# crockwell/far

Measured on AMD Instinct MI355X. Metric: image-pairs/sec (match+solve+regress) at 640x480, higher is better.
Workload: dtype f32

## Files before the change

### far_amd/csrc/conv_igemm_f16s.hip

```cpp
#include "common.h"
#include "linear_small.h"
#include <vector>
#include <type_traits>

namespace {

typedef _Float16 f16x8 __attribute__((ext_vector_type(8)));
typedef __attribute__((address_space(1))) const void* gptr_t;
typedef __attribute__((address_space(3))) void* lptr_t;

constexpr int TW = 16;
constexpr int A_PXB = 80;
constexpr int ACT_EXP_DEFAULT = 4;

template <int KS, int MW, int ST>
struct Geo {
    static constexpr int TH = 4 * MW;
    static constexpr int HW = ST * (TW - 1) + KS, HH = ST * (TH - 1) + KS;
    static constexpr int PX = KS == 1 ? 64 * MW : HW * HH;
    static constexpr int ROWB = KS == 1 ? 0 : (HW * A_PXB + 255) / 256 * 256;
    static constexpr int A_PLANE = KS == 1 ? PX * A_PXB : HH * ROWB;
    static constexpr int ITEMS = PX * 4;
    __device__ static constexpr int px_off(int hy, int hx) { return hy * ROWB + hx * A_PXB; }
};

struct ConvArgs {
    const float* x;
    const float* x2;
    int Cin1;
    const unsigned char* w;
    const float* zeros;
    const float* scale;
    const float* shift;
    const float* res;
    int res_group;
    const float* ln_gamma;
    const float* ln_beta;
    float ln_eps;
    const float* post_res;
    const float* up;
    float* y;
    long npix;
    long ntiles;
    int Csub;
    int H, W, Ho, Wo, Cin, Cout, tilesX, tilesY, nchunks, nblkY, act;
    float slope;
    float act_scale;
    float out_mul;
    int* overflow;
    const float* scale_dev;
    float* kv_part;
    int kv_S, kv_valid;
    const unsigned char* kv_img;
    float la_eps, la_vlen;
    int sub2;
    const long* g_b;
    const long* g_cell;
    int g_wc, g_W, g_stride, g_Hf, g_Wf;
};

__device__ __forceinline__ void split8(const float4& u, const float4& v, float act_scale, f16x8& hi, f16x8& lo) {
    const float x[8] = {u.x, u.y, u.z, u.w, v.x, v.y, v.z, v.w};
#pragma unroll
    for (int i = 0; i < 8; i += 2) {
        f16x2 h, l;
        split2(f32x2{x[i], x[i + 1]} * f32x2{act_scale, act_scale}, h, l);
        hi[i] = h.x; hi[i + 1] = h.y;
        lo[i] = l.x; lo[i + 1] = l.y;
    }
}

typedef float f32x4 __attribute__((ext_vector_type(4)));
template <int ITERS>
struct Stage {
    f32x4 v[ITERS][2];
};

struct TilePos {
    int img, oy0, ox0;
    long pix0;
};

template <int KS, int MW, int ST, int NTHR, int ITERS>
__device__ __forceinline__ void stage_pixels(int (&pixv)[ITERS], const ConvArgs& p, const TilePos& tp, int tid) {
    using G = Geo<KS, MW, ST>;
#pragma unroll
    for (int it = 0; it < ITERS; ++it) {
        const int i = tid + NTHR * it;
        const int hp = i >> 2;
        const int hy = hp / G::HW, hx = hp - hy * G::HW;
        const int iy = ST * tp.oy0 - KS / 2 + hy, ix = ST * tp.ox0 - KS / 2 + hx;
        const bool ok = i < G::ITEMS && iy >= 0 && iy < p.H && ix >= 0 && ix < p.W;
        pixv[it] = ok ? (tp.img * p.H + iy) * p.W + ix : -1;
    }
}

template <int KS, int MW, int ST, int NTHR, int ITERS>
__device__ __forceinline__ void stage_load(Stage<ITERS>& st, const ConvArgs& p, const TilePos& tp, int chunk, int tid, bool live = true,
                                           const int* rowpix = nullptr, const int* pixv = nullptr) {
    using G = Geo<KS, MW, ST>;
#pragma unroll
    for (int it = 0; it < ITERS; ++it) {
        const int i = tid + NTHR * it;
        const int hp = i >> 2, g = i & 3;
        const int c0 = 32 * chunk + 8 * g;
        bool ok = live && i < G::ITEMS;
        long pix;
        if (KS != 1 && pixv) {
            pix = pixv[it];
            ok = live && pixv[it] >= 0;
        } else if (KS == 1) {
            pix = tp.pix0 + hp;
            ok = ok && pix < p.npix;
            if (rowpix) {
                const int gp = rowpix[hp < 64 * MW ? hp : 0];
                pix = gp;
                ok = ok && gp >= 0;
            } else if (p.sub2) {
                const unsigned up = (unsigned)pix, rowg = up / (unsigned)p.Wo, ox = up - rowg * (unsigned)p.Wo;
                const unsigned n = rowg / (unsigned)p.Ho, oy = rowg - n * (unsigned)p.Ho;
                pix = ((long)n * p.H + 2 * oy) * p.W + 2 * ox;
            }
        } else {
            const int hy = hp / G::HW, hx = hp - hy * G::HW;
            const int iy = ST * tp.oy0 - KS / 2 + hy, ix = ST * tp.ox0 - KS / 2 + hx;
            ok = ok && iy >= 0 && iy < p.H && ix >= 0 && ix < p.W;
            pix = ((long)tp.img * p.H + iy) * p.W + ix;
        }
        const bool ok0 = ok && c0 < p.Cin, ok1 = ok && c0 + 4 < p.Cin;
#if defined(FAR_K9_EXP) && (FAR_K9_EXP & 4)
        pix &= 1023;
#endif
        const bool second = c0 >= p.Cin1;
        const float* base = second ? p.x2 + pix * (p.Cin - p.Cin1) + (c0 - p.Cin1) : p.x + pix * p.Cin1 + c0;
#if defined(FAR_K9_EXP) && (FAR_K9_EXP & 1)
        const float* src0 = p.zeros;
        const float* src1 = p.zeros;
        (void)base; (void)ok0; (void)ok1;
#else
        const float* src0 = ok0 ? base : p.zeros;
        const float* src1 = ok1 ? base + 4 : p.zeros;
#endif
        asm volatile("global_load_dwordx4 %0, %1, off" : "=v"(st.v[it][0]) : "v"(src0) : "memory");
        asm volatile("global_load_dwordx4 %0, %1, off" : "=v"(st.v[it][1]) : "v"(src1) : "memory");
    }
}

template <int YOUNGER, int ITERS>
__device__ __forceinline__ void stage_arrived(Stage<ITERS>& st) {
    static_assert(YOUNGER >= 0 && YOUNGER < 64, "vmcnt is a 6-bit counter");
    asm volatile("s_waitcnt vmcnt(%0)" : : "n"(YOUNGER) : "memory");
#pragma unroll
    for (int it = 0; it < ITERS; ++it) {
        f32x4 &u = st.v[it][0], &w = st.v[it][1];
        asm volatile("" : "+v"(u), "+v"(w));
    }
}

template <int KS, int MW, int ST, int NTHR, int ITERS, bool SPLIT>
__device__ __forceinline__ void stage_store(const Stage<ITERS>& st, unsigned char* As, int tid, float act_scale) {
    using G = Geo<KS, MW, ST>;
#pragma unroll
    for (int it = 0; it < ITERS; ++it) {
        const int i = tid + NTHR * it;
        const float4 u = make_float4(st.v[it][0].x, st.v[it][0].y, st.v[it][0].z, st.v[it][0].w);
        const float4 w = make_float4(st.v[it][1].x, st.v[it][1].y, st.v[it][1].z, st.v[it][1].w);
        if (ITERS * NTHR == G::ITEMS || i < G::ITEMS) {
            const int hp = i >> 2, g = i & 3;
            int off;
            if (KS == 1) off = hp * A_PXB;
            else { const int hy = hp / G::HW; off = G::px_off(hy, hp - hy * G::HW); }
            f16x8 hi, lo;
            split8(u, w, act_scale, hi, lo);
            *reinterpret_cast<f16x8*>(As + off + g * 16) = hi;
            if (SPLIT) *reinterpret_cast<f16x8*>(As + G::A_PLANE + off + g * 16) = lo;
        }
    }
}

template <int KS, int NTW>
__device__ __forceinline__ void conv_epilogue(const ConvArgs& p, const f32x16 (&acc)[2][NTW], const TilePos& tp,
                                              int cout_w, int wm, int l31, int h) {
    const float* __restrict__ resp = p.res;
    float* __restrict__ yp = p.y;
    const int rowstep = (KS == 1 ? 16 : p.Wo) * p.Csub;
#pragma unroll
    for (int mt = 0; mt < 2; ++mt) {
        const int mtile = 2 * wm + mt;
        long pix0;
        int nrow, ncol;
        if (KS == 1) {
            pix0 = tp.pix0 + 32 * mtile;
            const long left = p.npix - pix0;
            nrow = left >= 32 ? 2 : (left > 16 ? 2 : (left > 0 ? 1 : 0));
            ncol = left >= 32 ? 16 : -1;
        } else {
            const int oy = tp.oy0 + 2 * mtile;
            pix0 = ((long)tp.img * p.Ho + oy) * p.Wo + tp.ox0;
            nrow = p.Ho - oy;
            ncol = p.Wo - tp.ox0;
        }
        const long left = KS == 1 ? p.npix - pix0 : 0;
        int delta[16];
        bool ok[16];
#pragma unroll
        for (int r = 0; r < 16; ++r) {
            const int trow = r >> 3, tcol = (r & 3) + 8 * ((r >> 2) & 1) + 4 * h;
            delta[r] = trow * rowstep + tcol * p.Csub;
            ok[r] = (KS == 1 && ncol < 0) ? (16 * trow + tcol < left) : (trow < nrow && tcol < ncol);
        }
#pragma unroll
        for (int nt = 0; nt < NTW; ++nt) {
            const int co = cout_w + 32 * nt + l31;
            if (co >= p.Cout) continue;
            const float sc = p.scale[co] * p.out_mul, sh = p.shift ? p.shift[co] : 0.f;
            const int plane = co / p.Csub;
            const long base = (long)plane * p.npix * p.Csub + pix0 * p.Csub + (co - plane * p.Csub);
            float rv[16];
#pragma unroll
            for (int r = 0; r < 16; ++r) {
                rv[r] = 0.f;
                if (resp && ok[r]) {
                    if (p.res_group > 1) {
                        const long pix = pix0 + 16 * (r >> 3) + ((r & 3) + 8 * ((r >> 2) & 1) + 4 * h);
                        rv[r] = resp[(pix / p.res_group) * p.Cout + co];
                    } else {
                        rv[r] = resp[base + delta[r]];
                    }
                }
            }
#pragma unroll
            for (int r = 0; r < 16; ++r) {
                float v = acc[mt][nt][r] * sc + sh + rv[r];
                if (p.act == 1) v = fmaxf(v, 0.f);
                else if (p.act == 2) v = v > 0.f ? v : v * p.slope;
                if (ok[r]) yp[base + delta[r]] = v;
            }
        }
    }
}

#if defined(FAR_K9_EXP) && (FAR_K9_EXP & 8)
#define FAR_K9_STORE4(ptr, val) __builtin_nontemporal_store(f32x4{(val).x, (val).y, (val).z, (val).w}, reinterpret_cast<f32x4*>(ptr))
#else
#define FAR_K9_STORE4(ptr, val) (*reinterpret_cast<float4*>(ptr) = (val))
#endif

#ifdef FAR_K9_TIMING
__device__ unsigned long long g_k9_stamps[12 * 65536];
#define FAR_K9_STAMP(i) do { if (threadIdx.x == 0 && blockIdx.x < 65536) g_k9_stamps[12 * blockIdx.x + (i)] = __builtin_amdgcn_s_memtime(); } while (0)
#else
#define FAR_K9_STAMP(i) do {} while (0)
#endif

#define FAR_DPP_F(v, ctrl) __builtin_bit_cast(float, __builtin_amdgcn_update_dpp(0, __builtin_bit_cast(int, v), ctrl, 0xF, 0xF, true))
__device__ __forceinline__ float sum32(float v) {
    v += FAR_DPP_F(v, 0xB1);
    v += FAR_DPP_F(v, 0x4E);
    v += FAR_DPP_F(v, 0x141);
    v += FAR_DPP_F(v, 0x140);
    return v + shfl_xor_f(v, 16);
}

__device__ __forceinline__ void arrived(float4& v) { asm volatile("" : "+v"(v.x), "+v"(v.y), "+v"(v.z), "+v"(v.w)); }

template <int KS, int NW, int UP>
__device__ __forceinline__ void conv_epilogue_wide(const ConvArgs& p, const f32x16 (&acc)[2][4], const TilePos& tp,
                                                   int cout_w, int wm, int wave, int lane, float* lw, float* xch,
                                                   int mask_mt = -1, int mask_lo = 0, int mask_hi = 0) {
    const int l31 = lane & 31, h = lane >> 5;
    const float* __restrict__ resp = p.res;
    float* __restrict__ yp = p.y;
    float sc[4], sh[4];
#pragma unroll
    for (int nt = 0; nt < 4; ++nt) {
        const int co = cout_w + 32 * nt + l31;
        sc[nt] = co < p.Cout ? p.scale[co] * p.out_mul : 0.f;
        sh[nt] = (co < p.Cout && p.shift) ? p.shift[co] : 0.f;
    }
    const int co4 = cout_w + 4 * l31;
    const bool cok_all = co4 < p.Cout;
    const bool lane_masked = l31 >= mask_lo && l31 < mask_hi;
    const int plane = cok_all ? co4 / p.Csub : 0;
    const long cbase = (long)plane * p.npix * p.Csub + (co4 - plane * p.Csub);
#pragma unroll
    for (int mt = 0; mt < 2; ++mt) {
        const bool cok = cok_all && !(mt == mask_mt && lane_masked);
        const int mtile = 2 * wm + mt;
        long pix0;
        int nrow, ncol;
        long left = 0;
        if (KS == 1) {
            pix0 = tp.pix0 + 32 * mtile;
            left = p.npix - pix0;
            nrow = 2; ncol = 16;
        } else {
            const int oy = tp.oy0 + 2 * mtile;
            pix0 = ((long)tp.img * p.Ho + oy) * p.Wo + tp.ox0;
            nrow = p.Ho - oy;
            ncol = p.Wo - tp.ox0;
        }
#pragma unroll
        for (int nt = 0; nt < 4; ++nt)
#pragma unroll
// ... 875 lines not shown
            float v = 0.f;
            if (n < Cout && ch < Cin) v = w[(long)n * s_co + (long)ch * s_ci + (long)tap * s_tap] * wmul;
            const _Float16 hh = (_Float16)v;
            dst[e] = hh;
            if (planes == 2) dst[(size_t)NT * 16 + e] = (_Float16)(v - (float)hh);
        }
    }
}

struct PackRow {
    const float* w;
    long s_co, s_ci, s_tap;
    int Cin, Cout, taps, nchunks, nblkY, NT, planes, owns_scale;
    const float* w_all;
    long n_all;
    float* pack_scale;
    _Float16* out;
    const float* base_scale;
    float* scale_vec;
};
__device__ AmaxSlot g_pack_slots[4096];

__global__ __launch_bounds__(256) void k_pack_table_scales(const PackRow* __restrict__ rows) {
    const PackRow r = rows[blockIdx.y];
    if (!r.owns_scale) return;
    __shared__ unsigned part[256];
    unsigned m = 0;
    for (long i = (long)blockIdx.x * 256 + threadIdx.x; i < r.n_all; i += (long)gridDim.x * 256) {
        const unsigned b = __float_as_uint(fabsf(r.w_all[i]));
        m = b > m ? b : m;
    }
    part[threadIdx.x] = m;
    __syncthreads();
    for (int d = 128; d >= 1; d >>= 1) {
        if ((int)threadIdx.x < d && part[threadIdx.x + d] > part[threadIdx.x]) part[threadIdx.x] = part[threadIdx.x + d];
        __syncthreads();
    }
    if (threadIdx.x == 0) {
        AmaxSlot* const sl = g_pack_slots + (blockIdx.y & 4095);
        atomicMax(&sl->max_bits, part[0]);
        __threadfence();
        if (atomicAdd(&sl->ticket, 1u) == gridDim.x - 1) {
            __threadfence();
            const unsigned bits = atomicExch(&sl->max_bits, 0u);
            atomicExch(&sl->ticket, 0u);
            write_scales<0>(__uint_as_float(bits), r.pack_scale);
        }
    }
}

__global__ __launch_bounds__(256) void k_pack_table_images(const PackRow* __restrict__ rows) {
    const PackRow r = rows[blockIdx.y];
    const float wmul = r.pack_scale[0];
    if (r.scale_vec && blockIdx.x == 0)
        for (int co = threadIdx.x; co < r.Cout; co += 256) r.scale_vec[co] = (r.base_scale ? r.base_scale[co] : 1.0f) * r.pack_scale[1];
    const long total = (long)r.taps * r.nchunks * 2 * r.nblkY * r.NT * 2;
    if (blockIdx.x == 0 && threadIdx.x < 16) r.out[(size_t)total * 8 * r.planes + threadIdx.x] = (_Float16)0.f;
    for (long i = (long)blockIdx.x * 256 + threadIdx.x; i < total; i += (long)gridDim.x * 256) {
        long t = i;
        const int s = (int)(t & 1); t >>= 1;
        const int nn = (int)(t % r.NT); t /= r.NT;
        const int by = (int)(t % r.nblkY); t /= r.nblkY;
        const int ks = (int)(t & 1); t >>= 1;
        const int tap = (int)(t % r.taps);
        const int chunk = (int)(t / r.taps);
        const int n = by * r.NT + nn;
        const size_t row = r.planes == 2 ? ((((size_t)(chunk * r.taps + tap) * 2 + ks) * r.nblkY + by) * 2) * r.NT + nn
                                         : ((((size_t)(chunk * r.taps + tap) * r.nblkY + by) * 2 + ks)) * r.NT + nn;
        _Float16* dst = r.out + row * 16 + ((s ^ ((nn >> 3) & 1)) * 8);
        for (int e = 0; e < 8; ++e) {
            const int ch = 32 * chunk + 16 * ks + 8 * s + e;
            float v = 0.f;
            if (n < r.Cout && ch < r.Cin) v = r.w[(long)n * r.s_co + (long)ch * r.s_ci + (long)tap * r.s_tap] * wmul;
            const _Float16 hh = (_Float16)v;
            dst[e] = hh;
            if (r.planes == 2) dst[(size_t)r.NT * 16 + e] = (_Float16)(v - (float)hh);
        }
    }
}

struct TileCfg { int mw, nw, nt; };
inline TileCfg cfg_for(int Cout, int stride) {
    const int pad128 = (Cout + 127) / 128 * 128, pad256 = (Cout + 255) / 256 * 256;
    return (stride == 1 && pad128 < pad256) ? TileCfg{4, 1, 128} : TileCfg{2, 2, 256};
}

template <int KS, int MW, int NW, int NTW, bool SPLIT, int ST = 1, int UP = 0, bool N7 = false, int EPI = 0>
int launch_conv(const ConvArgs& a, dim3 grid, hipStream_t stream) {
    using G = Geo<KS, MW, ST>;
    constexpr int PLANES = SPLIT ? 2 : 1;
    constexpr int smem_loop = PLANES * G::A_PLANE + 3 * 2 * 32 * NTW * NW * 32;
    constexpr int smem_epi = EPI == 2 ? MW * NW * 32 * LDW * 4
                                      : MW * NW * (32 * 128 * 4 + 32 * 4);
    constexpr int smem_need = smem_loop + (EPI != 0 ? 64 * MW * 4 : 0);
    constexpr int smem = smem_need > smem_epi ? smem_need : smem_epi;
    bool cfg_failed = false;
    FAR_ONCE_PER_DEVICE(cfg_failed = hipFuncSetAttribute((const void*)k_conv<KS, MW, NW, NTW, SPLIT, ST, UP, N7, EPI>,
                                                         hipFuncAttributeMaxDynamicSharedMemorySize, smem) != hipSuccess);
    if (cfg_failed) return far_check_launch();
    hipLaunchKernelGGL((k_conv<KS, MW, NW, NTW, SPLIT, ST, UP, N7, EPI>), grid, dim3(64 * MW * NW), smem, stream, a);
    return far_check_launch();
}

template <int KS, bool SPLIT>
int launch_cfg(const TileCfg& c, const ConvArgs& a, dim3 grid, hipStream_t stream, bool small = false) {
    if (KS == 1 && a.up) {
        const bool rowwise = (a.Wo & 31) == 0 && far_get_tuning(13) == 0;
        if (c.mw == 4) return rowwise ? launch_conv<1, 4, 1, 4, SPLIT, 1, 2>(a, grid, stream) : launch_conv<1, 4, 1, 4, SPLIT, 1, 1>(a, grid, stream);
        return rowwise ? launch_conv<1, 2, 2, 4, SPLIT, 1, 2>(a, grid, stream) : launch_conv<1, 2, 2, 4, SPLIT, 1, 1>(a, grid, stream);
    }
    if constexpr (KS == 1) {
        if (c.mw == 2 && small) return launch_conv<1, 1, 2, 4, SPLIT>(a, grid, stream);
        if (c.mw == 4 && small) return launch_conv<1, 2, 1, 4, SPLIT>(a, grid, stream);
    }
    if (c.mw == 4) return launch_conv<KS, 4, 1, 4, SPLIT>(a, grid, stream);
    if constexpr (KS == 3) {
        if (a.nblkY == 1 && a.Cout > 192 && a.Cout <= 224 && ((a.Cout | a.Csub) & 3) == 0 && far_get_tuning(4) == 0)
            return launch_conv<KS, 2, 2, 4, SPLIT, 1, false, true>(a, grid, stream);
    }
    return launch_conv<KS, 2, 2, 4, SPLIT>(a, grid, stream);
}

template <bool SPLIT>
int launch_stride2(const ConvArgs& a, dim3 grid, hipStream_t stream) { return launch_conv<3, 2, 2, 4, SPLIT, 2>(a, grid, stream); }

}

extern "C" {

int far_weight_scale_f32(const float* w, long n, float* scale_out, hipStream_t stream);
int far_conv_pack_view_f32(const float* w, long s_co, long s_ci, long s_tap, int Cin, int Cout, int ksize, int stride, int split,
                           const float* scale_in, void* packed, hipStream_t stream);
int far_conv_pack_view_scaled_f32(const float* w, long s_co, long s_ci, long s_tap, int Cin, int Cout, int ksize, int stride, int split,
                                  const float* scale_in, void* packed, const float* base_scale, float* scale_vec_out,
                                  hipStream_t stream);

size_t far_conv_packed_bytes(int Cin, int Cout, int ksize, int stride, int split) {
    if (Cin <= 0 || Cout <= 0 || (ksize != 1 && ksize != 3) || stride < 1 || stride > 2 || (stride == 2 && ksize != 3)) return 0;
    const int NT = cfg_for(Cout, stride).nt;
    const size_t nchunks = (Cin + 31) / 32, nblkY = (Cout + NT - 1) / NT;
    return (size_t)ksize * ksize * nchunks * nblkY * (split ? 2 : 1) * NT * 64 + 32;
}

int far_conv_pack_f32(const float* w, int Cin, int Cout, int ksize, int stride, int w_exp, int split, void* packed,
                      hipStream_t stream) {
    far_clear_errors();
    if (!w || !packed || far_conv_packed_bytes(Cin, Cout, ksize, stride, split) == 0 || w_exp < -60 || w_exp > 60) return FAR_EINVAL;
    const int NT = cfg_for(Cout, stride).nt;
    const int nchunks = (Cin + 31) / 32, nblkY = (Cout + NT - 1) / NT;
    hipLaunchKernelGGL(k_conv_pack, dim3(512), dim3(256), 0, stream, w, (long)Cin * ksize * ksize, (long)ksize * ksize, 1L, Cin, Cout,
                       ksize * ksize, nchunks, nblkY, NT, split ? 2 : 1, ldexpf(1.0f, w_exp), (const float*)nullptr, (_Float16*)packed);
    return far_check_launch();
}

int far_weight_scale_f32(const float* w, long n, float* scale_out, hipStream_t stream) {
    far_clear_errors();
    if (!w || !scale_out || n <= 0) return FAR_EINVAL;
    if ((reinterpret_cast<uintptr_t>(w) & 15) == 0) {
        launch_amax_scale<0>(w, n, scale_out, stream);
    } else {
        hipMemsetAsync(scale_out, 0, 2 * sizeof(float), stream);
        hipLaunchKernelGGL(k_absmax_bits, dim3(256), dim3(256), 0, stream, w, n, reinterpret_cast<unsigned*>(scale_out));
        hipLaunchKernelGGL(k_pack_scale, dim3(1), dim3(1), 0, stream, scale_out);
    }
    return far_check_launch();
}

int far_conv_pack_view_f32(const float* w, long s_co, long s_ci, long s_tap, int Cin, int Cout, int ksize, int stride, int split,
                           const float* scale_in, void* packed, hipStream_t stream) {
    return far_conv_pack_view_scaled_f32(w, s_co, s_ci, s_tap, Cin, Cout, ksize, stride, split, scale_in, packed, nullptr, nullptr, stream);
}

int far_conv_pack_view_scaled_f32(const float* w, long s_co, long s_ci, long s_tap, int Cin, int Cout, int ksize, int stride, int split,
                                  const float* scale_in, void* packed, const float* base_scale, float* scale_vec_out,
                                  hipStream_t stream) {
    far_clear_errors();
    if (!w || !packed || !scale_in || far_conv_packed_bytes(Cin, Cout, ksize, stride, split) == 0) return FAR_EINVAL;
    const int NT = cfg_for(Cout, stride).nt;
    const int nchunks = (Cin + 31) / 32, nblkY = (Cout + NT - 1) / NT;
    const long items = (long)ksize * ksize * nchunks * 2 * nblkY * NT * 2;
    long blocks = (items + 255) / 256;
    blocks = blocks < 1 ? 1 : (blocks > 512 ? 512 : blocks);
    hipLaunchKernelGGL(k_conv_pack, dim3((unsigned)blocks), dim3(256), 0, stream, w, s_co, s_ci, s_tap, Cin, Cout, ksize * ksize, nchunks, nblkY, NT,
                       split ? 2 : 1, 1.0f, scale_in, (_Float16*)packed, base_scale, scale_vec_out);
    return far_check_launch();
}

int far_conv_pack_auto_f32(const float* w, int Cin, int Cout, int ksize, int stride, int split, void* packed, float* scale_out,
                           hipStream_t stream) {
    far_clear_errors();
    if (!w || !packed || !scale_out || far_conv_packed_bytes(Cin, Cout, ksize, stride, split) == 0) return FAR_EINVAL;
    const long n = (long)Cout * Cin * ksize * ksize;
    const int rc = far_weight_scale_f32(w, n, scale_out, stream);
    if (rc != FAR_OK) return rc;
    return far_conv_pack_view_f32(w, (long)Cin * ksize * ksize, (long)ksize * ksize, 1, Cin, Cout, ksize, stride, split, scale_out,
                                  packed, stream);
}

__global__ void k_grad_scale(float* __restrict__ s) {
    const float amax = s[0];
    int e = 0;
    if (amax > 0.f && amax <= FLT_MAX) (void)frexpf(amax, &e);
    int ex = 10 - e;
    ex = ex < -100 ? -100 : (ex > 100 ? 100 : ex);
    s[0] = ldexpf(1.0f, ex);
    s[1] = ldexpf(1.0f, ACT_EXP_DEFAULT - ex);
}
int far_grad_scale_f32(const float* x, long n, float* out2, hipStream_t stream) {
    far_clear_errors();
    if (!x || !out2 || n <= 0) return FAR_EINVAL;
    if ((reinterpret_cast<uintptr_t>(x) & 15) == 0) {
        launch_amax_scale<1>(x, n, out2, stream);
    } else {
        hipMemsetAsync(out2, 0, 2 * sizeof(float), stream);
        hipLaunchKernelGGL(k_absmax_bits, dim3(256), dim3(256), 0, stream, x, n, reinterpret_cast<unsigned*>(out2));
        hipLaunchKernelGGL(k_grad_scale, dim3(1), dim3(1), 0, stream, out2);
    }
    return far_check_launch();
}

struct far_conv_desc {
    const float* x;
    const float* x2;
    const void* packed;
    const float* scale;
    const float* shift;
    const float* res;
    const float* ln_gamma;
    const float* ln_beta;
    const float* post_res;
    const float* up;
    float* y;
    long N;
    int H, W, Cin, Cin1, Cout, ksize, stride;
    int act, split, out_planes, res_group;
    float slope, ln_eps;
    int act_exp;
    int* overflow;
    const float* act_scale_dev;
};

}

namespace {
struct KvMode {
    int epi;
    float* part;
    int S, valid;
    const unsigned char* img;
    float eps, vlen;
    const long *g_b = nullptr, *g_cell = nullptr;
    int g_wc = 0, g_W = 0, g_stride = 0, g_Hf = 0, g_Wf = 0;
};

int conv_nhwc_impl(const far_conv_desc* desc, const KvMode* kvm, hipStream_t stream) {
    if (!desc) return FAR_EINVAL;
    const far_conv_desc& d = *desc;
    const float *x = d.x, *x2 = d.x2, *scale = d.scale, *shift = d.shift, *res = d.res;
    const float *ln_gamma = d.ln_gamma, *ln_beta = d.ln_beta, *post_res = d.post_res, *up = d.up;
    const void* packed = d.packed;
    float* y = d.y;
    const long N = d.N;
    const int H = d.H, W = d.W, Cin = d.Cin, Cin1 = d.Cin1, Cout = d.Cout, ksize = d.ksize, stride = d.stride;
    const int act = d.act, split = d.split, out_planes = d.out_planes, res_group = d.res_group;
    const float slope = d.slope, ln_eps = d.ln_eps;
    far_clear_errors();
    if (d.act_exp < -24 || d.act_exp > 8) return FAR_EINVAL;
    if (N == 0) return FAR_OK;
    const bool sub2 = ksize == 1 && stride == 2;
    const int pstride = sub2 ? 1 : stride;
    if (!x || !packed || !scale || (!y && !(kvm && kvm->epi == 1)) || N < 0 || H <= 0 || W <= 0 || Cin <= 0 || (Cin & 3) || Cout <= 0 ||
        (ksize != 1 && ksize != 3) || stride < 1 || stride > 2 || act < 0 || act > 2 ||
        (sub2 && (kvm || up || x2 || res_group != 1 || N * (long)((H - 1) / 2 + 1) * ((W - 1) / 2 + 1) > 0x7fffffffL)) ||
        (ksize == 3 && N * (long)H * W > 0x7fffffffL) ||
        (act == 2 && !(slope >= 0.f && slope <= 1.f)) || x == y || (x2 && x2 == y) || out_planes < 1 || Cout % out_planes)
        return FAR_EINVAL;
    if (res_group < 1 || (res_group > 1 && (!res || ksize != 1 || out_planes != 1 || (N * H * W) % res_group))) return FAR_EINVAL;
    if (x2 ? (Cin1 <= 0 || Cin1 >= Cin || (Cin1 & 7)) : (Cin1 != Cin)) return FAR_EINVAL;
    if (up && (ksize != 1 || (H & 1) || (W & 1) || W < 32 || out_planes != 1 || res || ln_gamma || post_res || (Cout & 3) ||
               up == y || (long)(H / 2) * (W / 2) * Cout > 0x7fffffffL))
        return FAR_EINVAL;
    ConvArgs a;
    a.x = x; a.x2 = x2; a.Cin1 = Cin1; a.w = (const unsigned char*)packed; a.scale = scale;
    a.zeros = reinterpret_cast<const float*>((const unsigned char*)packed + far_conv_packed_bytes(Cin, Cout, ksize, pstride, split) - 32); a.shift = shift; a.res = res; a.res_group = res_group; a.y = y;
    a.ln_gamma = ln_gamma; a.ln_beta = ln_beta; a.ln_eps = ln_eps; a.post_res = post_res; a.up = up;
    a.H = H; a.W = W; a.Ho = (H - 1) / stride + 1; a.Wo = (W - 1) / stride + 1; a.Cin = Cin; a.Cout = Cout; a.Csub = Cout / out_planes;
    a.npix = N * a.Ho * a.Wo;
    if (kvm && kvm->epi != 3 && kvm->valid != kvm->S) a.npix = a.npix / kvm->valid * kvm->S;
    const TileCfg c = cfg_for(Cout, pstride);
    if ((ln_gamma || post_res) && (!ln_gamma || !ln_beta || Cout != c.nt || out_planes != 1 || (Cout & 3) || post_res == y))
        return FAR_EINVAL;
    const int th = 4 * c.mw;
    a.tilesX = (a.Wo + TW - 1) / TW; a.tilesY = (a.Ho + th - 1) / th;
    a.nchunks = (Cin + 31) / 32;
    a.nblkY = (Cout + c.nt - 1) / c.nt;
    a.act = act; a.slope = slope;
    a.act_scale = ldexpf(1.0f, d.act_exp); a.out_mul = ldexpf(1.0f, ACT_EXP_DEFAULT - d.act_exp); a.overflow = d.overflow;
    a.scale_dev = d.act_scale_dev;
    a.kv_part = kvm ? kvm->part : nullptr; a.kv_S = kvm ? kvm->S : 0; a.kv_valid = kvm ? kvm->valid : 0;
    a.sub2 = sub2 ? 1 : 0;
    a.g_b = a.g_cell = nullptr; a.g_wc = a.g_W = a.g_stride = a.g_Hf = a.g_Wf = 0;
    a.kv_img = kvm ? kvm->img : nullptr; a.la_eps = kvm ? kvm->eps : 0.f; a.la_vlen = kvm ? kvm->vlen : 0.f;
    long nbx = ksize == 1 ? (a.npix + 64 * c.mw - 1) / (64 * c.mw) : N * a.tilesX * a.tilesY;
    if (ksize == 1 && !sub2 && !kvm && !up && !x2 && !ln_gamma && !post_res && res_group == 1 && split && nbx * a.nblkY < 512 &&
        far_get_tuning(7) == 0 && far_linear_small_covers(a.npix, Cin, Cout)) {
        LinSmallArgs s;
        s.x = x; s.w = a.w; s.scale = scale; s.shift = shift; s.res = res; s.y = y; s.rows = a.npix;
        s.Cin = Cin; s.Cout = Cout; s.Csub = a.Csub; s.NT = c.nt; s.nblkY = a.nblkY; s.act = act; s.slope = slope;
        s.act_scale = a.act_scale; s.out_mul = a.out_mul; s.scale_dev = a.scale_dev; s.overflow = a.overflow;
        return far_linear_small_launch(s, stream);
    }
    const bool small = ksize == 1 && !up && nbx * a.nblkY < 192 && far_get_tuning(7) == 0;
    if (small) nbx = (a.npix + 32 * c.mw - 1) / (32 * c.mw);
    a.ntiles = nbx;
    if (nbx * a.nblkY > 0x7fffffffL) return FAR_EINVAL;
    dim3 grid((unsigned)(nbx * a.nblkY));
    if (stride == 2 && ksize == 3) return split ? launch_stride2<true>(a, grid, stream) : launch_stride2<false>(a, grid, stream);
    if (ksize == 3) return split ? launch_cfg<3, true>(c, a, grid, stream) : launch_cfg<3, false>(c, a, grid, stream);
    if (kvm && kvm->epi == 3) {
        if (!split) return FAR_EINVAL;
        a.g_b = kvm->g_b; a.g_cell = kvm->g_cell; a.g_wc = kvm->g_wc; a.g_W = kvm->g_W; a.g_stride = kvm->g_stride;
        a.g_Hf = kvm->g_Hf; a.g_Wf = kvm->g_Wf;
        if (small) { nbx = (a.npix + 64 * c.mw - 1) / (64 * c.mw); a.ntiles = nbx; grid = dim3((unsigned)(nbx * a.nblkY)); }
        return c.mw == 4 ? launch_conv<1, 4, 1, 4, true, 1, 0, false, 3>(a, grid, stream)
                         : launch_conv<1, 2, 2, 4, true, 1, 0, false, 3>(a, grid, stream);
    }
    if (kvm) {
        if (c.mw != 2) return FAR_EINVAL;
        if (!split) {
            if (kvm->epi == 2)
                return small ? launch_conv<1, 1, 2, 4, false, 1, false, false, 2>(a, grid, stream)
                             : launch_conv<1, 2, 2, 4, false, 1, false, false, 2>(a, grid, stream);
            return small ? launch_conv<1, 1, 2, 4, false, 1, false, false, 1>(a, grid, stream)
                         : launch_conv<1, 2, 2, 4, false, 1, false, false, 1>(a, grid, stream);
        }
        if (kvm->epi == 2)
            return small ? launch_conv<1, 1, 2, 4, true, 1, false, false, 2>(a, grid, stream)
                         : launch_conv<1, 2, 2, 4, true, 1, false, false, 2>(a, grid, stream);
        return small ? launch_conv<1, 1, 2, 4, true, 1, false, false, 1>(a, grid, stream)
                     : launch_conv<1, 2, 2, 4, true, 1, false, false, 1>(a, grid, stream);
    }
    return split ? launch_cfg<1, true>(c, a, grid, stream, small) : launch_cfg<1, false>(c, a, grid, stream, small);
}
}

extern "C" {

int far_conv_nhwc_f32(const far_conv_desc* desc, hipStream_t stream) { return conv_nhwc_impl(desc, nullptr, stream); }

size_t far_linear_kv_workspace_bytes(long rows, int S) {
    if (rows <= 0 || S < 64 || rows % S) return 0;
    return (size_t)(rows / S) * ((S + 63) / 64) * 256 * 33 * sizeof(float);
}
size_t far_linear_kv_image_bytes(long n_img) { return n_img > 0 ? (size_t)n_img * KV_IMG_BYTES : 0; }

int far_linear_kv_f16s(const far_conv_desc* desc, int S, void* ws, float* kv, void* kv_img, hipStream_t stream) {
    if (!desc) return FAR_EINVAL;
    const far_conv_desc& d = *desc;
    far_clear_errors();
    const long rows = d.N * d.H * d.W;
    if (rows == 0) return FAR_OK;
    if (!ws || !kv || S < 64 || rows < 0 || rows % S || d.ksize != 1 || d.stride != 1 || d.Cout != 512 ||
        d.out_planes != 2 || d.act != 0 || d.res || d.ln_gamma || d.post_res || d.up || d.x2 || d.res_group != 1 || rows / S > 65535 ||
        d.act_scale_dev)
        return FAR_EINVAL;
    const int Sp = (S + 63) / 64 * 64;
    if (rows / S * (long)Sp > 0x7fffffffL) return FAR_EINVAL;
    KvMode m{1, (float*)ws, Sp, S, nullptr, 0.f, 0.f};
    const int rc = conv_nhwc_impl(desc, &m, stream);
    if (rc != FAR_OK) return rc;
    const int per = 256 * 33;
    hipLaunchKernelGGL(k_kv_blocks_reduce, dim3((per + 255) / 256, (unsigned)(rows / S)), dim3(256), 0, stream, (const float*)ws, Sp,
                       per, kv, (unsigned char*)kv_img, ldexpf(1.0f, d.act_exp));
    return far_check_launch();
}

int far_linear_q_apply_f16s(const far_conv_desc* desc, int L, int S, const void* kv_img, float eps, hipStream_t stream) {
    if (!desc) return FAR_EINVAL;
    const far_conv_desc& d = *desc;
    far_clear_errors();
    const long rows = d.N * d.H * d.W;
    if (rows == 0) return FAR_OK;
    if (!kv_img || !d.y || L < 64 || S <= 0 || rows < 0 || rows % L || d.ksize != 1 || d.stride != 1 ||
        d.Cout != 256 || d.out_planes != 1 || d.act != 0 || d.res || d.ln_gamma || d.post_res || d.up || d.x2 || d.res_group != 1 ||
        d.act_scale_dev)
        return FAR_EINVAL;
    const int Lp = (L + 63) / 64 * 64;
    if (rows / L * (long)Lp > 0x7fffffffL) return FAR_EINVAL;
    KvMode m{2, nullptr, Lp, L, (const unsigned char*)kv_img, eps, (float)S};
    return conv_nhwc_impl(desc, &m, stream);
}

int far_linear_gather_f16s(const far_conv_desc* desc, const int64_t* b_ids, const int64_t* cell_ids, int wc, int W, int stride,
                           long n_img, int Hf, int Wf, hipStream_t stream) {
    if (!desc) return FAR_EINVAL;
    const far_conv_desc& d = *desc;
    far_clear_errors();
    const long rows = d.N * d.H * d.W;
    if (rows == 0) return FAR_OK;
    if (!b_ids || !cell_ids || wc <= 0 || W <= 0 || W > 15 || stride <= 0 || n_img <= 0 || Hf <= 0 || Wf <= 0 || rows < 0 ||
        rows % (W * W) || rows > 0x7fffffffL || n_img * Hf * (long)Wf > 0x7fffffffL || d.ksize != 1 || d.stride != 1 || !d.split ||
        d.x2 || d.up || d.ln_gamma || d.post_res || d.act_scale_dev || d.out_planes != 1)
        return FAR_EINVAL;
    KvMode m{3, nullptr, 0, 0, nullptr, 0.f, 0.f};
    m.g_b = reinterpret_cast<const long*>(b_ids); m.g_cell = reinterpret_cast<const long*>(cell_ids);
    m.g_wc = wc; m.g_W = W; m.g_stride = stride; m.g_Hf = Hf; m.g_Wf = Wf;
    return conv_nhwc_impl(desc, &m, stream);
}

struct far_pack_item {
    const float* w;
    long s_co, s_ci, s_tap;
    int Cin, Cout, ksize, stride, split, scale_owner;
    const float* w_all;
    long n_all;
    float* pack_scale;
    void* packed;
    const float* base_scale;
    float* scale_vec;
};
long far_pack_table_bytes(int n) { return n > 0 ? (long)n * (long)sizeof(PackRow) : 0; }

int far_pack_table_build(const far_pack_item* items, int n, void* table_dev, hipStream_t stream) {
    far_clear_errors();
    if (!items || !table_dev || n <= 0 || n > 4096) return FAR_EINVAL;
    std::vector<PackRow> rows((size_t)n);
    for (int i = 0; i < n; ++i) {
        const far_pack_item& it = items[i];
        if (!it.w || !it.packed || !it.pack_scale || it.scale_owner < 0 || it.scale_owner >= n ||
            far_conv_packed_bytes(it.Cin, it.Cout, it.ksize, it.stride, it.split) == 0)
            return FAR_EINVAL;
        const bool owns = it.scale_owner == i;
        if (owns ? (!it.w_all || it.n_all <= 0) : (items[it.scale_owner].pack_scale != it.pack_scale)) return FAR_EINVAL;
        PackRow& r = rows[(size_t)i];
        const int NT = cfg_for(it.Cout, it.stride).nt;
        r.w = it.w; r.s_co = it.s_co; r.s_ci = it.s_ci; r.s_tap = it.s_tap;
        r.Cin = it.Cin; r.Cout = it.Cout; r.taps = it.ksize * it.ksize; r.nchunks = (it.Cin + 31) / 32; r.nblkY = (it.Cout + NT - 1) / NT;
        r.NT = NT; r.planes = it.split ? 2 : 1; r.owns_scale = owns ? 1 : 0;
        r.w_all = it.w_all; r.n_all = it.n_all; r.pack_scale = it.pack_scale; r.out = (_Float16*)it.packed;
        r.base_scale = it.base_scale; r.scale_vec = it.scale_vec;
    }
    if (hipMemcpyAsync(table_dev, rows.data(), rows.size() * sizeof(PackRow), hipMemcpyHostToDevice, stream) != hipSuccess)
        return far_check_launch();
    return FAR_OK;
}

int far_pack_table_run(const void* table_dev, int n, hipStream_t stream) {
    far_clear_errors();
    if (!table_dev || n <= 0 || n > 4096) return FAR_EINVAL;
    const PackRow* rows = reinterpret_cast<const PackRow*>(table_dev);
    hipLaunchKernelGGL(k_pack_table_scales, dim3(16, (unsigned)n), dim3(256), 0, stream, rows);
    hipLaunchKernelGGL(k_pack_table_images, dim3(32, (unsigned)n), dim3(256), 0, stream, rows);
    return far_check_launch();
}

#ifdef FAR_K9_TIMING
__global__ void k_tick_probe(unsigned long long ticks, unsigned long long* out) {
    const unsigned long long t0 = __builtin_amdgcn_s_memtime(), r0 = __builtin_amdgcn_s_memrealtime();
    unsigned long long t1;
    do { t1 = __builtin_amdgcn_s_memtime(); } while (t1 - t0 < ticks);
    out[0] = t1 - t0; out[1] = __builtin_amdgcn_s_memrealtime() - r0;
}
int far_k9_tick_probe(unsigned long long ticks, unsigned long long* host2) {
    unsigned long long* d;
    if (hipMalloc(&d, 16) != hipSuccess) return -5;
    hipLaunchKernelGGL(k_tick_probe, dim3(1), dim3(64), 0, 0, ticks, d);
    hipMemcpy(host2, d, 16, hipMemcpyDeviceToHost);
    hipFree(d);
    return 0;
}
int far_k9_timing_dump(void* host, int nblocks) {
    return hipMemcpyFromSymbol(host, HIP_SYMBOL(g_k9_stamps), (size_t)nblocks * 12 * sizeof(unsigned long long)) == hipSuccess ? 0 : -5;
}
#endif

}
```

### far_amd/flags.py

```python
import os
from collections import namedtuple

Switch = namedtuple('Switch', 'env module attr off_value neutral scope doc')
SWITCHES = [
    Switch('FAR_NO_WINO', 'far_amd.ops', 'USE_WINO', False, 'parity', 'inference',
           'stride-1 3x3 convolutions on K9 (direct implicit GEMM) instead of K17 (Winograd F(2x2,3x3)); same operator, other summation'),
    Switch('FAR_NO_PAD', 'far_amd.loftr.backbone', 'PAD_CHANNELS', False, 'bitwise', 'inference',
           'the 196-channel backbone maps stored with 196 channels instead of 208 (zero weights for the extra ones: exact zeros)'),
    Switch('FAR_NO_PREFETCH', 'far_amd.loftr.model:LoFTR', 'head_prefetch', False, 'bitwise', 'inference',
           "the head's feature stage computed inside forward_rt_prediction instead of enqueued behind K1"),
    Switch('FAR_NO_SIDE_STREAM', 'far_amd.loftr.model:LoFTR', 'head_side_stream', False, 'bitwise', 'inference',
           "the head's feature stage on the step's own stream behind K1 (rounds 2-5) instead of on a second stream next to K1 and the fine level"),
    Switch('FAR_FPN_STREAM', 'far_amd.loftr.model:LoFTR', 'fpn_side_stream', True, 'bitwise', 'inference',
           "OPT-IN (1 switches it ON; default off): the FPN's fine branch on a side stream next to the coarse transformer and K1 (-0.6 ms per 32 "
           "pairs; off by default because the roofline launch -- K17 208 -> 208 @ 240x320 -- then shares the GPU and its in-step duration "
           "in a kernel trace is no longer its own)"),
    Switch('FAR_NO_GATHER_FUSE', 'far_amd.loftr.stages:FinePreprocess', 'fused_gather', False, 'bitwise', 'inference',
           'FinePreprocess.merge_feat on a materialised window tensor (K3 gather + K9) instead of K9 reading through the match indices'),
    Switch('FAR_NO_KV', 'far_amd.loftr.transformer:LoFTREncoderLayer', 'fused_kv', False, 'parity', 'inference',
           "k, v projections + K5's first half as separate launches instead of K9's k|v epilogue (the K'^T V sum changes order)"),
    Switch('FAR_NO_QAPPLY', 'far_amd.loftr.transformer:LoFTREncoderLayer', 'fused_apply', False, 'parity', 'inference',
           "q projection + K5's second half as separate launches instead of K9's attention-apply epilogue (q no longer stays in split operands)"),
    Switch('FAR_NO_STACK', 'far_amd.loftr.transformer:LocalFeatureTransformer', 'stack_self', False, 'bitwise', 'inference',
           "the two 'self' calls of an encoder layer on the two images separately instead of one call on both"),
    Switch('FAR_NO_BN', 'far_amd.ops', 'USE_HIP_BATCHNORM_TRAIN', False, 'parity', 'training',
           'training-mode BatchNorm on nn.BatchNorm2d + torch activations instead of K19 (tests/test_train_kernels_gpu.py holds K19 to the module)'),
]

ENV_ONLY = {
    'FAR_HIP_LIB': ('load', 'path of another build of libfar_hip.so (tools/ab_build.py: same-box A/B against a git revision); skips the build-id check'),
    'FAR_TUNING': ('load', 'comma-separated key=value pairs handed to far_set_tuning at load time, e.g. FAR_TUNING="10=1,8=1" (keys below)'),
    'FAR_SKIP_ASM_CHECK': ('build', "1: far_amd/build.py does not scan the generated code (K9's asm pixel loads; the LDS-DMA ring rule of every kernel with global_load_lds; the half-register writes of the asm fp16 split) after recompiling"),
    'FAR_EXTRA_HIPCC_FLAGS': ('build', 'extra hipcc flags of an experiment build (-DFAR_WINO_EXP=..., tools/wino_exp.sh); part of the build id'),
    'FAR_COMMIT': ('tools', 'commit stamp tools/collect_profiles.sh / tools/step_floors.py write into the profile files'),
    'FAR_C3_PY_NODE': ('bench', "bench.py --workload c3: the encoder layer's autograd node driven from Python instead of far_enc_layer_fwd / _bwd"),
    'FAR_C3_NO_OVERLAP': ('bench', 'bench.py --workload c3: the layer node without side streams'),
    'FAR_C3_PER_OP': ('bench', 'bench.py --workload c3: one autograd node per operator instead of per layer'),
    'FAR_TORCH_ADAMW': ('bench', 'bench.py --workload c3: torch.optim.AdamW instead of K20'),
    'FAR_CUDNN_BENCHMARK': ('bench', 'bench.py: torch.backends.cudnn.benchmark for the vendor comparison legs'),
}

Tuning = namedtuple('Tuning', 'key default values neutral doc')
TUNING = [
    Tuning(0, 3, (0, 1, 2, 4, 7), 'bitwise', 'bit mask of exact-f32 kernels that stagger wave-slot priorities: 1 k_stats, 2 k_match, 4 k_emm_pv'),
    Tuning(1, 0, (1,), 'parity', 'K1 exact-f32 variant: the other tile shape (another summation order of the row statistics)'),
    Tuning(2, 0, (1,), 'bitwise', 'conf_matrix writer variant A (store pattern)'),
    Tuning(3, 0, (1,), 'bitwise', 'conf_matrix writer variant B (store pattern)'),
    Tuning(4, 0, (1,), 'bitwise', 'K9 without the seven-tile mode / K5 windows on the generic path'),
    Tuning(5, 0, (1, 2, 4), 'bitwise', 'K5 apply: tiles per unit'),
    Tuning(6, 0, (64, 256), 'parity', "K5: tokens per K'^T V chunk (another partial-sum grouping)"),
    Tuning(7, 0, (1,), 'bitwise', 'K9 Linear launches always on full-height tiles'),
    Tuning(8, 0, (1,), 'bitwise', 'K17 splits its operands with the five-instruction split2 instead of v_fma_mix (same values)'),
    Tuning(9, 0, (1,), 'bitwise', 'K17 runs a short last channel block on the full body'),
    Tuning(10, 0, (1,), 'bitwise', "K1's match pass without the tile prescreen"),
    Tuning(11, 0, (1, 2), 'bitwise', "K14's pipeline: 0 = 4 waves / 3 slots / counted waits, two workgroups per CU; 1 = 8 waves / 4 slots / counted, one per CU (round 5's form); 2 = 4 waves / 3 slots / vmcnt(0) per phase (fallback without a wait table)"),
    Tuning(12, 0, (1,), 'parity', "K10's inference form on the exact-f32 matrix instruction instead of split fp16"),
    Tuning(15, 0, (1,), 'bitwise', 'K17: 1 = the multiplying wave group does NOT raise its issue priority (the round-4 kernel)'),
    Tuning(13, 0, (1,), 'bitwise', "K9's FPN-merge epilogue in its generic form everywhere"),
]


def off(env):
    if env not in {s.env for s in SWITCHES}:
        raise KeyError(f'{env} is not a registered far_amd switch (far_amd/flags.py)')
    return os.environ.get(env, '0') not in ('', '0')


def value(env, default=None):
    if env not in ENV_ONLY:
        raise KeyError(f'{env} is not a registered far_amd environment variable (far_amd/flags.py)')
    return os.environ.get(env, default)


def known():
    return {s.env for s in SWITCHES} | set(ENV_ONLY)


def unknown_in_environment():
    skip = ('FAR_WINO_', 'FAR_K9_')
    return sorted(k for k in os.environ if k.startswith('FAR_') and k not in known() and not k.startswith(skip))


def target(sw):
    import importlib
    mod, _, cls = sw.module.partition(':')
    obj = importlib.import_module(mod)
    return (getattr(obj, cls) if cls else obj), sw.attr
```

Measured before the change: 377.9.

## Add weight-resident persistent 1x1 conv kernel for split-fp16 launches

Adds a persistent 1x1 convolution kernel that loads the whole weight block into LDS once per workgroup and streams 32-pixel tiles through it, prefetching the next tile's activations while the current one computes and prefetching the epilogue residual/upsample operands. Eligible K9 1x1 launches (single channel block, no fused attention/LN epilogues) route to it by default; the FPN-merge upsample path stays on K9 unless tuning 14=2. It aims to cut repeated weight reloads and per-tile launch overhead. The cost is a large LDS footprint that limits occupancy, plus a grid capped at the CU count.

```diff
diff --git a/far_amd/csrc/conv1x1_stream.h b/far_amd/csrc/conv1x1_stream.h
--- /dev/null
+++ b/far_amd/csrc/conv1x1_stream.h
@@ -0,0 +1,20 @@
+#pragma once
+#include "common.h"
+
+struct Conv1x1StreamArgs {
+    const float* x;
+    const unsigned char* w;
+    const float* zeros;
+    const float* scale;
+    const float* shift;
+    const float* res;
+    const float* up;
+    float* y;
+    long npix;
+    int H, W, Ho, Wo, Cin, Cout, NT, sub2, act;
+    float slope, act_scale, out_mul;
+    int* overflow;
+};
+
+bool far_conv1x1_stream_covers(int Cin, int Cout);
+int far_conv1x1_stream_launch(const Conv1x1StreamArgs& a, hipStream_t stream);
diff --git a/far_amd/csrc/conv1x1_stream_f16s.hip b/far_amd/csrc/conv1x1_stream_f16s.hip
--- /dev/null
+++ b/far_amd/csrc/conv1x1_stream_f16s.hip
@@ -0,0 +1,291 @@
+#include "conv1x1_stream.h"
+
+namespace {
+
+typedef _Float16 f16x8 __attribute__((ext_vector_type(8)));
+
+constexpr int MAX_KS = 8;
+constexpr int MAX_NT = 7;
+constexpr int EPI_LD = 72;
+constexpr int EPI_WAVE_BYTES = 32 * EPI_LD * 4;
+constexpr int LDS_MAX = 160 * 1024;
+constexpr int PB = 4;
+
+__device__ __forceinline__ void split8(const f32x4& u, const f32x4& v, float act_scale, f16x8& hi, f16x8& lo) {
+    const float x[8] = {u.x, u.y, u.z, u.w, v.x, v.y, v.z, v.w};
+#pragma unroll
+    for (int i = 0; i < 8; i += 2) {
+        f16x2 h, l;
+        split2(f32x2{x[i], x[i + 1]} * f32x2{act_scale, act_scale}, h, l);
+        hi[i] = h.x; hi[i + 1] = h.y;
+        lo[i] = l.x; lo[i + 1] = l.y;
+    }
+}
+
+__device__ __forceinline__ void arrived(f32x4& v) { asm volatile("" : "+v"(v)); }
+
+template <int MODE, int NKS, int NTL>
+__global__ __launch_bounds__(256) void k_conv1x1_stream(const Conv1x1StreamArgs p) {
+    extern __shared__ __attribute__((aligned(16))) unsigned char smem[];
+    const int tid = threadIdx.x, lane = tid & 63, wave = tid >> 6, l31 = lane & 31, h = lane >> 5;
+    const int nks = (p.Cin + 15) >> 4;
+    constexpr int ntp = 32 * NTL, NPASS = (NTL + 1) / 2;
+    unsigned char* const Ws = smem;
+    float* const lw = reinterpret_cast<float*>(smem + NKS * 2 * ntp * 32 + wave * EPI_WAVE_BYTES);
+
+    {
+        constexpr int units = NKS * 2 * ntp * 2;
+        for (int u = tid; u < units; u += 256) {
+            const int rowu = u % (ntp * 2), sp = u / (ntp * 2);
+            const bool have = sp < 2 * nks;
+            const uint4 v = *reinterpret_cast<const uint4*>(have ? p.w + ((size_t)sp * p.NT * 2 + rowu) * 16 : (const unsigned char*)p.zeros);
+            *reinterpret_cast<uint4*>(Ws + (size_t)u * 16) = v;
+        }
+    }
+    float* const scs = reinterpret_cast<float*>(smem + NKS * 2 * ntp * 32 + 4 * EPI_WAVE_BYTES), * const shs = scs + ntp;
+    if (tid < ntp) {
+        scs[tid] = tid < p.Cout ? p.scale[tid] * p.out_mul : 0.f;
+        shs[tid] = (tid < p.Cout && p.shift) ? p.shift[tid] : 0.f;
+    }
+    __syncthreads();
+    const unsigned char* const bfrag = Ws + l31 * 32 + ((h ^ ((l31 >> 3) & 1)) * 16);
+    const float as = p.act == 2 ? p.slope : 0.f, ab = p.act == 0 ? -__builtin_inff() : 0.f;
+
+    const long ntiles = (p.npix + 31) >> 5;
+    const long tstep = (long)gridDim.x * 4;
+
+    f32x4 raw[NKS][2];
+    auto request = [&](long t) {
+        const long pix = 32 * t + l31;
+        const bool ok = t < ntiles && pix < p.npix;
+        long src = pix;
+        if (p.sub2) {
+            const unsigned up = (unsigned)pix, rowg = up / (unsigned)p.Wo, ox = up - rowg * (unsigned)p.Wo;
+            const unsigned n = rowg / (unsigned)p.Ho, oy = rowg - n * (unsigned)p.Ho;
+            src = ((long)n * p.H + 2 * oy) * p.W + 2 * ox;
+        }
+        const float* base = p.x + (ok ? src * p.Cin + 8 * h : 0);
+#pragma unroll
+        for (int k = 0; k < NKS; ++k) {
+            const bool live = ok && k < nks;
+            const float* s = live ? base + 16 * k : p.zeros;
+            raw[k][0] = *reinterpret_cast<const f32x4*>(s);
+            raw[k][1] = *reinterpret_cast<const f32x4*>(s + 4);
+        }
+    };
+
+    const long t0 = (long)blockIdx.x * 4 + wave;
+    request(t0);
+    f16x8 ah[NKS], al[NKS];
+#pragma unroll
+    for (int k = 0; k < NKS; ++k) split8(raw[k][0], raw[k][1], p.act_scale, ah[k], al[k]);
+    for (long t = t0; t < ntiles; t += tstep) {
+        request(t + tstep);
+
+        const long pix0 = 32 * t;
+        const int left = p.npix - pix0 >= 32 ? 32 : (int)(p.npix - pix0);
+        const int g = lane >> 4, c16 = lane & 15;
+
+
+        f32x16 acc[NTL];
+#pragma unroll
+        for (int nt = 0; nt < NTL; ++nt)
+#pragma unroll
+            for (int r = 0; r < 16; ++r) acc[nt][r] = 0.f;
+        constexpr int NG = 4, GPK = (NTL + NG - 1) / NG, NGRP = NKS * GPK;
+        f16x8 bh[2][NG], bl[2][NG];
+        auto read_b = [&](int grp) {
+            const int k = grp / GPK, n0 = NG * (grp % GPK);
+#pragma unroll
+            for (int q = 0; q < NG; ++q) {
+                if (n0 + q >= NTL) continue;
+                const unsigned char* B = bfrag + ((size_t)(2 * k) * ntp + 32 * (n0 + q)) * 32;
+                bh[grp & 1][q] = *reinterpret_cast<const f16x8*>(B);
+                bl[grp & 1][q] = *reinterpret_cast<const f16x8*>(B + (size_t)ntp * 32);
+            }
+        };
+        read_b(0);
+#pragma unroll
+        for (int grp = 0; grp < NGRP; ++grp) {
+            const int k = grp / GPK, n0 = NG * (grp % GPK), s = grp & 1;
+            if (grp + 1 < NGRP) read_b(grp + 1);
+#pragma unroll
+            for (int q = 0; q < NG; ++q)
+                if (n0 + q < NTL) acc[n0 + q] = __builtin_amdgcn_mfma_f32_32x32x16_f16(ah[k], bh[s][q], acc[n0 + q], 0, 0, 0);
+#pragma unroll
+            for (int q = 0; q < NG; ++q)
+                if (n0 + q < NTL) acc[n0 + q] = __builtin_amdgcn_mfma_f32_32x32x16_f16(ah[k], bl[s][q], acc[n0 + q], 0, 0, 0);
+#pragma unroll
+            for (int q = 0; q < NG; ++q)
+                if (n0 + q < NTL) acc[n0 + q] = __builtin_amdgcn_mfma_f32_32x32x16_f16(al[k], bh[s][q], acc[n0 + q], 0, 0, 0);
+            __builtin_amdgcn_sched_barrier(0);
+        }
+
+        const float* eptr[8];
+        unsigned dxm = 0, dym = 0;
+        float wy[8], wx[8];
+        if (MODE == 2) {
+            const int hc = p.Ho >> 1, wc = p.Wo >> 1;
+            const float ry = p.Ho > 1 ? (float)(hc - 1) / (float)(p.Ho - 1) : 0.f;
+            const float rx = p.Wo > 1 ? (float)(wc - 1) / (float)(p.Wo - 1) : 0.f;
+            const long per = (long)p.Ho * p.Wo;
+            const long n0 = pix0 / per;
+            const int rem = (int)(pix0 - n0 * per);
+            const int Y0 = rem / p.Wo, X0 = rem - Y0 * p.Wo;
+#pragma unroll
+            for (int it = 0; it < 8; ++it) {
+                const int q = 4 * it + g;
+                int X = X0 + q, Y = Y0;
+                long n = n0;
+                if (X >= p.Wo) { X -= p.Wo; ++Y; }
+                if (Y >= p.Ho) { Y = 0; ++n; }
+                const float sy = ry * (float)Y, sx = rx * (float)X;
+                const int y0 = (int)sy, x0 = (int)sx;
+                const int y1 = y0 + (y0 < hc - 1 ? 1 : 0), x1 = x0 + (x0 < wc - 1 ? 1 : 0);
+                wy[it] = sy - (float)y0; wx[it] = sx - (float)x0;
+                const bool ok = q < left;
+                eptr[it] = p.up + (ok ? (n * hc * (long)wc) * p.Cout + (long)(y0 * wc + x0) * p.Cout : 0);
+                dxm |= (ok && x1 != x0) ? 1u << it : 0u;
+                dym |= (ok && y1 != y0) ? 1u << it : 0u;
+            }
+        } else if (MODE == 1) {
+#pragma unroll
+            for (int it = 0; it < 8; ++it) {
+                const int q = 4 * it + g;
+                eptr[it] = p.res + (q < left ? (pix0 + q) * p.Cout : 0);
+            }
+        }
+        constexpr int NE = MODE == 2 ? 4 : 1;
+        f32x4 E[2][PB][NE];
+        auto issue = [&](int b) {
+            if (MODE == 0) return;
+            const int c4 = 64 * (b >> 1) + 4 * c16;
+            const int coff = c4 < p.Cout ? c4 : 0;
+#pragma unroll
+            for (int j = 0; j < PB; ++j) {
+                const int it = PB * (b & 1) + j;
+                const float* s = eptr[it] + coff;
+                E[b & 1][j][0] = *reinterpret_cast<const f32x4*>(s);
+                if (MODE == 2) {
+                    const int dxo = (dxm >> it) & 1u ? p.Cout : 0, dyo = (dym >> it) & 1u ? (p.Wo >> 1) * p.Cout : 0;
+                    E[b & 1][j][1] = *reinterpret_cast<const f32x4*>(s + dxo);
+                    E[b & 1][j][2] = *reinterpret_cast<const f32x4*>(s + dyo);
+                    E[b & 1][j][3] = *reinterpret_cast<const f32x4*>(s + dyo + dxo);
+                }
+            }
+        };
+        issue(0);
+
+        if (p.overflow) {
+            float chk = 0.f;
+#pragma unroll
+            for (int nt = 0; nt < NTL; ++nt)
+#pragma unroll
+                for (int r = 0; r < 16; ++r) chk += acc[nt][r];
+            const bool bad = !(fabsf(chk) <= FLT_MAX);
+            if (__any(bad) && lane == 0) atomicOr(p.overflow, 1);
+        }
+
+#pragma unroll
+        for (int k = 0; k < NKS; ++k) split8(raw[k][0], raw[k][1], p.act_scale, ah[k], al[k]);
+
+#pragma unroll
+        for (int pass = 0; pass < NPASS; ++pass) {
+#pragma unroll
+            for (int j = 0; j < 2; ++j) {
+                const int nt = 2 * pass + j;
+                if (nt >= NTL) continue;
+                const float sc = scs[32 * nt + l31], sh = shs[32 * nt + l31];
+#pragma unroll
+                for (int r = 0; r < 16; ++r) {
+                    const int q = 16 * (r >> 3) + (r & 3) + 8 * ((r >> 2) & 1) + 4 * h;
+                    lw[q * EPI_LD + 32 * j + l31] = acc[nt][r] * sc + sh;
+                }
+            }
+            const int c4 = 64 * pass + 4 * c16;
+            const bool cok = c4 < p.Cout;
+            float* const ybase = p.y + (pix0 * (long)p.Cout + (cok ? c4 : 0));
+#pragma unroll
+            for (int half = 0; half < 2; ++half) {
+                const int b = 2 * pass + half;
+                if (b + 1 < 2 * NPASS) issue(b + 1);
+                f32x4 vv[PB];
+#pragma unroll
+                for (int j = 0; j < PB; ++j) vv[j] = *reinterpret_cast<const f32x4*>(lw + (4 * (PB * half + j) + g) * EPI_LD + 4 * c16);
+                if (MODE != 0) {
+#pragma unroll
+                    for (int j = 0; j < PB; ++j)
+#pragma unroll
+                        for (int e = 0; e < NE; ++e) arrived(E[b & 1][j][e]);
+                }
+#pragma unroll
+                for (int j = 0; j < PB; ++j) {
+                    const int it = PB * half + j, q = 4 * it + g;
+                    f32x4 v = vv[j];
+                    if (MODE == 1) {
+                        const f32x4 rr = E[b & 1][j][0];
+                        v.x += rr.x; v.y += rr.y; v.z += rr.z; v.w += rr.w;
+                    }
+                    if (MODE == 2) {
+                        const f32x4 ta = E[b & 1][j][0], tb = E[b & 1][j][1], tc = E[b & 1][j][2], td = E[b & 1][j][3];
+                        const float ly = wy[it], lx = wx[it], hy = 1.f - ly, hx = 1.f - lx;
+                        v.x += hy * (hx * ta.x + lx * tb.x) + ly * (hx * tc.x + lx * td.x);
+                        v.y += hy * (hx * ta.y + lx * tb.y) + ly * (hx * tc.y + lx * td.y);
+                        v.z += hy * (hx * ta.z + lx * tb.z) + ly * (hx * tc.z + lx * td.z);
+                        v.w += hy * (hx * ta.w + lx * tb.w) + ly * (hx * tc.w + lx * td.w);
+                    }
+                    v.x = fmaxf(v.x, __builtin_fmaf(v.x, as, ab)); v.y = fmaxf(v.y, __builtin_fmaf(v.y, as, ab));
+                    v.z = fmaxf(v.z, __builtin_fmaf(v.z, as, ab)); v.w = fmaxf(v.w, __builtin_fmaf(v.w, as, ab));
+                    if (cok && q < left) *reinterpret_cast<f32x4*>(ybase + (long)q * p.Cout) = v;
+                }
+                __builtin_amdgcn_sched_barrier(0);
+            }
+        }
+    }
+}
+
+template <int MODE, int NKS, int NTL>
+int launch(const Conv1x1StreamArgs& a, unsigned grid, hipStream_t stream) {
+    constexpr int smem = NKS * 2 * 32 * NTL * 32 + 4 * EPI_WAVE_BYTES + 2 * 32 * NTL * 4;
+    static_assert(smem <= LDS_MAX, "the operand image and the four transpose tiles share one CU's LDS");
+    bool cfg_failed = false;
+    FAR_ONCE_PER_DEVICE(cfg_failed = hipFuncSetAttribute((const void*)k_conv1x1_stream<MODE, NKS, NTL>,
+                                                         hipFuncAttributeMaxDynamicSharedMemorySize, smem) != hipSuccess);
+    if (cfg_failed) return far_check_launch();
+    hipLaunchKernelGGL((k_conv1x1_stream<MODE, NKS, NTL>), dim3(grid), dim3(256), smem, stream, a);
+    return far_check_launch();
+}
+
+template <int MODE>
+int launch_mode(const Conv1x1StreamArgs& a, unsigned grid, hipStream_t stream) {
+    const bool k8 = a.Cin > 64, n7 = a.Cout > 128;
+    if (k8) return n7 ? launch<MODE, 8, 7>(a, grid, stream) : launch<MODE, 8, 4>(a, grid, stream);
+    return n7 ? launch<MODE, 4, 7>(a, grid, stream) : launch<MODE, 4, 4>(a, grid, stream);
+}
+
+int cu_count() {
+    static std::atomic<int> cus[64];
+    const int dev = far_current_device();
+    int n = cus[dev].load(std::memory_order_relaxed);
+    if (n <= 0) {
+        if (hipDeviceGetAttribute(&n, hipDeviceAttributeMultiprocessorCount, dev) != hipSuccess || n <= 0) n = 256;
+        cus[dev].store(n, std::memory_order_relaxed);
+    }
+    return n;
+}
+
+}
+
+bool far_conv1x1_stream_covers(int Cin, int Cout) {
+    return Cin > 0 && (Cin & 15) == 0 && Cin <= 16 * MAX_KS && Cout > 0 && (Cout & 3) == 0 && Cout <= 32 * MAX_NT;
+}
+
+int far_conv1x1_stream_launch(const Conv1x1StreamArgs& a, hipStream_t stream) {
+    if (!far_conv1x1_stream_covers(a.Cin, a.Cout) || a.npix <= 0) return FAR_EINVAL;
+    const long ntiles = (a.npix + 31) / 32, want = (ntiles + 3) / 4;
+    const int cus = cu_count();
+    const unsigned grid = (unsigned)(want < cus ? want : cus);
+    if (a.up) return launch_mode<2>(a, grid, stream);
+    if (a.res) return launch_mode<1>(a, grid, stream);
+    return launch_mode<0>(a, grid, stream);
+}
diff --git a/far_amd/csrc/conv_igemm_f16s.hip b/far_amd/csrc/conv_igemm_f16s.hip
--- a/far_amd/csrc/conv_igemm_f16s.hip
+++ b/far_amd/csrc/conv_igemm_f16s.hip
@@ -1,5 +1,6 @@
 #include "common.h"
 #include "linear_small.h"
+#include "conv1x1_stream.h"
 #include <vector>
 #include <type_traits>
 
@@ -1481,6 +1482,16 @@
     a.g_b = a.g_cell = nullptr; a.g_wc = a.g_W = a.g_stride = a.g_Hf = a.g_Wf = 0;
     a.kv_img = kvm ? kvm->img : nullptr; a.la_eps = kvm ? kvm->eps : 0.f; a.la_vlen = kvm ? kvm->vlen : 0.f;
     long nbx = ksize == 1 ? (a.npix + 64 * c.mw - 1) / (64 * c.mw) : N * a.tilesX * a.tilesY;
+    const int stream_mode = far_get_tuning(14);
+    if (ksize == 1 && split && !kvm && !x2 && !ln_gamma && !post_res && !d.act_scale_dev && out_planes == 1 && res_group == 1 &&
+        a.nblkY == 1 && (H > 1 || up || sub2) && stream_mode != 1 && (!up || stream_mode == 2) &&
+        far_conv1x1_stream_covers(Cin, Cout)) {
+        Conv1x1StreamArgs s;
+        s.x = x; s.w = a.w; s.zeros = a.zeros; s.scale = scale; s.shift = shift; s.res = res; s.up = up; s.y = y; s.npix = a.npix;
+        s.H = H; s.W = W; s.Ho = a.Ho; s.Wo = a.Wo; s.Cin = Cin; s.Cout = Cout; s.NT = c.nt; s.sub2 = a.sub2; s.act = act;
+        s.slope = slope; s.act_scale = a.act_scale; s.out_mul = a.out_mul; s.overflow = a.overflow;
+        return far_conv1x1_stream_launch(s, stream);
+    }
     if (ksize == 1 && !sub2 && !kvm && !up && !x2 && !ln_gamma && !post_res && res_group == 1 && split && nbx * a.nblkY < 512 &&
         far_get_tuning(7) == 0 && far_linear_small_covers(a.npix, Cin, Cout)) {
         LinSmallArgs s;
diff --git a/far_amd/flags.py b/far_amd/flags.py
--- a/far_amd/flags.py
+++ b/far_amd/flags.py
@@ -57,6 +57,7 @@
     Tuning(12, 0, (1,), 'parity', "K10's inference form on the exact-f32 matrix instruction instead of split fp16"),
     Tuning(15, 0, (1,), 'bitwise', 'K17: 1 = the multiplying wave group does NOT raise its issue priority (the round-4 kernel)'),
     Tuning(13, 0, (1,), 'bitwise', "K9's FPN-merge epilogue in its generic form everywhere"),
+    Tuning(14, 0, (1, 2), 'bitwise', "the weight-resident 1x1 kernel (K9s, conv1x1_stream_f16s.hip): 1 = off, its launches run on K9; 2 = it also takes the FPN-merge launches (`up`; slower than K9 there, off by default)"),
 ]
 
 
```

New measurement: 378.3 (median of 4 runs). About the same (+0.1%).
